# iosefa/obia

Measured on AMD Instinct MI355X. Metric: Mpixel/s (SLIC+zonal feats) on 16384²×8-band; achieved HBM GB/s fraction, higher is better.
Workload: dtype f32

## Files before the change

obia_amd/csrc/slic.hip:

```cpp
#include "slic.hpp"
#include "slic_features.hpp"

#include <cmath>
#include <cstdlib>

namespace obia {

void regular_grid_hw(long long H, long long W, long long n, long long out[4]) {
    long long dims[3] = {1, H, W};
    int order[3] = {0, 1, 2};
    for (int i = 0; i < 3; ++i)
        for (int j = i + 1; j < 3; ++j)
            if (dims[order[j]] < dims[order[i]]) std::swap(order[i], order[j]);
    double sd[3];
    for (int i = 0; i < 3; ++i) sd[i] = (double)dims[order[i]];
    double space = sd[0] * sd[1] * sd[2];
    if (space <= (double)n) { out[0] = out[1] = out[2] = out[3] = 0; return; }
    double st[3];
    for (int i = 0; i < 3; ++i) st[i] = std::pow(space / (double)n, 1.0 / 3.0);
    auto all_ge = [&]() { return sd[0] >= st[0] && sd[1] >= st[1] && sd[2] >= st[2]; };
    if (!all_ge()) {
        for (int d = 0; d < 3; ++d) {
            st[d] = sd[d];
            double sp = 1.0;
// ... 688 lines not shown
    __syncthreads();
    if (threadIdx.x == 0) {
        const int tot = s_c[0] + s_c[1] + s_c[2] + s_c[3];
        if (tot) atomicAdd(&out[p], tot);
    }
}

int slic_plan_layout(obia_ctx *ctx, SlicBatch &b) {
    if (b.d_tile_prob) return OBIA_OK;
    const int np = b.nprob;
    long long tiles_all = 0;
    int tile_max = 0;
    for (int p = 0; p < np; ++p) {
        SlicProblem &P = b.probs[p];
        P.tiles_x = cdiv(P.W, SWEEP_TW);
        P.tiles_y = cdiv(P.H, SWEEP_TH);
        const int nt = P.tiles_x * P.tiles_y;
        if (tiles_all + nt > 0x7fff0000LL) { set_error("too many sweep tiles in one batch"); return OBIA_E_INVALID; }
        P.tile_off = (int)tiles_all;
        tiles_all += nt;
        if (nt > tile_max) tile_max = nt;
    }
    b.total_tiles_all = tiles_all > 0 ? tiles_all : 1;
    b.total_tiles = tile_max;
    std::vector<int> tp((size_t)b.total_tiles_all, 0);
    for (int p = 0; p < np; ++p)
        for (int t = 0; t < b.probs[p].tiles_x * b.probs[p].tiles_y; ++t) tp[(size_t)b.probs[p].tile_off + t] = p;
    b.d_probs = ctx->plan.add(ctx, b.probs.data(), (size_t)np);
    b.d_tile_prob = ctx->plan.add(ctx, tp.data(), tp.size());
    if (!b.d_probs || !b.d_tile_prob) return OBIA_E_NOMEM;
    return OBIA_OK;
}

int slic_count_valid(obia_ctx *ctx, SlicBatch &b, std::vector<int> &nvalid, int *d_cnt_cleared) {
    const int np = b.nprob;
    Arena &A = ctx->arena;
    nvalid.assign(np, 0);
    OBIA_TRY(slic_plan_layout(ctx, b));
    if (b.masked) {
        OBIA_TRY(ctx->plan.flush(ctx));
        int *d_cnt = d_cnt_cleared;
        if (!d_cnt) {
            d_cnt = A.get<int>(np);
            if (!d_cnt) return OBIA_E_NOMEM;
            OBIA_TRY(fill_async(ctx, d_cnt, 0, sizeof(int) * np));
        }
        int blocks = cdiv(b.maxpix, 256 * 16 * 32);
        if (blocks < 1) blocks = 1;
        hipLaunchKernelGGL(count_valid_kernel, dim3(blocks, np), dim3(256), 0, ctx->stream, b.d_probs, b.d_mask, d_cnt);
        OBIA_TRY(read_back(ctx, nvalid.data(), d_cnt, sizeof(int) * np));
    } else {
        for (int p = 0; p < np; ++p) nvalid[p] = b.probs[p].H * b.probs[p].W;
    }
    return OBIA_OK;
}

int slic_plan_and_seed(obia_ctx *ctx, SlicBatch &b, const std::vector<int> &n_segments, const std::vector<int> *nvalid_in,
                       const ExternalSeeds *ext) {
    const int np = b.nprob;
    if (ext)
        for (int p = 0; p < np; ++p)
            if (ext[p].n < 0 || (ext[p].n > 0 && !ext[p].yx && !ext[p].d_yx)) { set_error("external seeds of problem %d: bad set", p); return OBIA_E_INVALID; }
    Arena &A = ctx->arena;
    OBIA_TRY(slic_plan_layout(ctx, b));
    std::vector<int> nvalid;
    if (nvalid_in) nvalid = *nvalid_in;
    else OBIA_TRY(slic_count_valid(ctx, b, nvalid));
    if (ext && np == 1 && ext->n > 0 && nvalid[0] <= 0) { set_error("the mask has no valid pixel"); return OBIA_E_EMPTY; }
    std::vector<SeedGrid> grids(np);
    std::vector<double> stepmax(np);
    b.step.assign(np, 1.0f);
    b.grid_n.assign(np, 0);
    int cent_off = 0;
    for (int p = 0; p < np; ++p) {
// ... 149 lines not shown
```

obia_amd/csrc/slic.hpp:

```cpp
#pragma once
#include "common.hpp"

namespace obia {

struct SlicProblem {
    int H, W;
    int K;
    int sy, sx;
    int ncy, ncx;
    float spatial_w;
    int cent_off;
    int cell_off;
    int tile_off;
    int tiles_x, tiles_y;
    long long pix_off;
    long long feat_off;
    int XB;
    int n_valid;
    long long fb_off;
    float sp_y, sp_x;
    int direct;
    int m4_off;
};

// ... 101 lines not shown
    }
    return members;
}

struct SmoothSpec {
    double sigma[3] = {0.0, 0.0, 0.0};
    float *tmp_a = nullptr, *tmp_b = nullptr;
    double *d_w[3] = {nullptr, nullptr, nullptr};
    int radius[3] = {0, 0, 0};
    unsigned *d_scratch = nullptr;
    bool on() const { return sigma[0] > 1e-15 || sigma[1] > 1e-15 || sigma[2] > 1e-15; }
};
int smooth_prepare(obia_ctx *ctx, SmoothSpec &sm, long long total_pix, int CP, int np);
int gaussian_weights_host(double sigma, bool sigma_is_f32, std::vector<double> &w);
int slic_features_launch(hipStream_t stream, const SlicBatch &b, const float *src, int Ws, unsigned *d_keys, const SmoothSpec *smooth = nullptr,
                         bool minmax_only = false);
bool slic_fuse_features(const SlicBatch &b, const float *src, int Ws);
double slic_fscale(float maxabs);
int slic_features_finish(SlicBatch &b, const unsigned *keys, const unsigned *nonfinite, const unsigned *maxabs_bits, std::vector<int> *skip);
int slic_prepare_features(obia_ctx *ctx, SlicBatch &b, const float *src, int Ws, std::vector<int> *skip = nullptr);
float slic_prescale(float ratio, int normalize, int to_lab, bool slic_zero);
bool slic_use_colour_bound(float ratio, bool to_lab = false);
void slic_batch_settings(SlicBatch &b, const obia_slic_params &p, int C, int normalize_bands, bool masked);
int slic_batch_layout(SlicBatch &b);
inline std::pair<int, int> slic_cc_sizes(double min_size_factor, double max_size_factor, int n_valid, int K) {
    const double segment_size = K > 0 ? (double)n_valid / (double)K : 1.0;
    const double mxd = max_size_factor * segment_size;
    return {(int)(min_size_factor * segment_size), mxd >= 2147483647.0 ? 2147483647 : (mxd >= 1.0 ? (int)mxd : 1)};
}

struct ExternalSeeds { const double *yx; int n; double step; const float *d_yx = nullptr; };
int slic_plan_and_seed(obia_ctx *ctx, SlicBatch &b, const std::vector<int> &n_segments,
                       const std::vector<int> *nvalid = nullptr, const ExternalSeeds *ext = nullptr);
int slic_count_valid(obia_ctx *ctx, SlicBatch &b, std::vector<int> &nvalid, int *d_cnt_cleared = nullptr);
int slic_plan_layout(obia_ctx *ctx, SlicBatch &b);

int slic_run_sweeps(obia_ctx *ctx, SlicBatch &b);
int slic_sweeps_settle(obia_ctx *ctx, bool *repeat);
int slic_rerun_storing(obia_ctx *ctx, SlicBatch &b);

int slic_stage_outputs(obia_ctx *ctx, const SlicBatch &b, float *features, float *seeds_yx, float *centroids);

int mask_centroids_dev(obia_ctx *ctx, const uint8_t *mask, int H, int W, const int64_t *picks, int K, const int64_t *dense, long long n_dense,
                       int iters, double *centroids_yx_out, double *steps_zyx_out);
int mask_centroids_queue(obia_ctx *ctx, const uint8_t *mask, int h, int w, long long n_valid, const int64_t *picks, int K, const int64_t *dense,
                         long long n_dense, int iters, float *seeds_out_dev, double *steps_out_dev);

struct CcProblem { int H, W; long long pix_off; int min_size; int max_size; };
struct CcResolve { const int *parent; const int *newlab; const int *small_final; int start_label; int mask_label; };
#if defined(__HIPCC__)
__device__ __forceinline__ int cc_resolve_label(const CcResolve &R, long long i) {
    const int p = R.parent[i];
    if (p < 0) return R.mask_label;
    const int r = R.parent[p];
    int nl = R.newlab[r];
    if (nl < 0) nl = R.small_final[-nl - 2];
    return (nl >= 0) ? nl + R.start_label : 0;
}
#endif
int enforce_connectivity_batch(obia_ctx *ctx, const std::vector<CcProblem> &probs, const int32_t *labels_in,
                               long long total_pix, int start_label, int32_t *labels_out, int *h_n_labels_out,
                               CcResolve *deferred = nullptr, const CcProblem *d_probs = nullptr);

int enforce_connectivity_dev(obia_ctx *ctx, const int32_t *labels_in, int H, int W, int min_size,
                             int max_size, int start_label, int32_t *labels_out, int *d_n_labels_out);

int zonal_stats_dev(obia_ctx *ctx, const float *raw, const int32_t *labels, int H, int W, int C,
                    const int32_t *bands_host, int n_bands, int n_labels, int start_label,
                    int64_t *count, double *mean, double *var, float *mn, float *mx);
int zonal_moments_dev(obia_ctx *ctx, const float *raw, const int32_t *labels, int H, int W, int C,
                      const int32_t *bands_host, int n_bands, int n_labels, int start_label, const double *mean,
                      double *skew, double *kurt, double *var );

}
```

obia_amd/csrc/tiling.hip:

```cpp
#include "slic.hpp"
#include "../../include/obia_testing.h"

#include <cmath>
#include <cstdlib>

namespace obia {

struct TileWin { int y0, x0, h, w; long long pix_off; int cly, clx; int cly_in, clx_in, cly_any, clx_any; int m4_off; };

__device__ __forceinline__ void wave_hist_add(unsigned *hist, int key, bool active) {
    bool todo = active;
    while (true) {
        const unsigned long long act = __ballot(todo);
        if (!act) break;
        const int leader = __ffsll((long long)act) - 1;
        const int kk = __shfl(key, leader);
        const unsigned long long same = __ballot(todo && key == kk);
        if ((int)(threadIdx.x & 63) == leader) atomicAdd(&hist[kk], (unsigned)__popcll(same));
        if (key == kk) todo = false;
    }
}

__device__ __forceinline__ bool in_corner(const TileWin &t, int y, int x) {
    return (y >= t.h - t.cly) && (x < t.clx || x >= t.w - t.clx);
}
__device__ __forceinline__ bool wholly_in_corner(const TileWin &t, int y, int x) {
    return (y >= t.h - t.cly_in) && (x < t.clx_in || x >= t.w - t.clx_in);
}
__device__ __forceinline__ bool meets_corner(const TileWin &t, int y, int x) {
    return (y >= t.h - t.cly_any) && (x < t.clx_any || x >= t.w - t.clx_any);
}

__global__ __launch_bounds__(256) void tile_count_inside_kernel(const TileWin *__restrict__ wins, const int32_t *__restrict__ G,
                                                                int Wr, unsigned *__restrict__ inside, int *__restrict__ tile_any) {
    const TileWin t = wins[blockIdx.y];
    bool seen = false;
    const int wround = ((t.w + 255) / 256) * 256;
    for (int y = blockIdx.x; y < t.h; y += gridDim.x) {
        const bool low = y >= t.h - t.cly_any;
        for (int x0 = 0; x0 < wround; x0 += 4 * 256) {
            int g[4];
#pragma unroll
            for (int u = 0; u < 4; ++u) {
                const int x = x0 + 256 * u + threadIdx.x;
                g[u] = 0;
                if (x < t.w && !(low && wholly_in_corner(t, y, x))) {
                    g[u] = G[(long long)(t.y0 + y) * Wr + t.x0 + x];
                    seen |= g[u] > 0;
                    if (low && meets_corner(t, y, x)) g[u] = 0;
                }
            }
#pragma unroll
            for (int u = 0; u < 4; ++u)
                if (x0 + 256 * u < wround) wave_hist_add(inside, g[u], g[u] > 0);
        }
    }
    if (__ballot(seen) && (threadIdx.x & 63) == 0) tile_any[blockIdx.y] = 1;
}

template <bool VEC4>
__global__ __launch_bounds__(256) void tile_mask_kernel(const TileWin *__restrict__ wins, const uint8_t *__restrict__ inmask,
                                                        int32_t *__restrict__ G, int Wr, int white,
                                                        const unsigned *__restrict__ inside, const unsigned *__restrict__ seg_size,
                                                        uint8_t *__restrict__ alive, uint8_t *__restrict__ dmask,
                                                        const int *__restrict__ tile_any, unsigned *__restrict__ dmask4) {
    const TileWin t = wins[blockIdx.y];
    if (white && tile_any[blockIdx.y] == 0) white = 0;
    auto decide = [&](int y, int x, long long gp, uint8_t m, int g) -> uint8_t {
        if (!white) return m;
        if (in_corner(t, y, x)) return 0;
        if (g > 0) {
            if (inside[g] == seg_size[g]) { G[gp] = 0; alive[g] = 0; }
            else m = 0;
        }
        return m;
    };
    if (VEC4) {
        const int w4 = t.w >> 2, nq = (t.h + 3) >> 2;
        for (int q = blockIdx.x; q < nq; q += gridDim.x)
            for (int x4 = threadIdx.x; x4 < w4; x4 += 256) {
                const int x = 4 * x4;
                unsigned mw[4];
                int4 g[4];
#pragma unroll
                for (int j = 0; j < 4; ++j) {
                    const int y = 4 * q + j;
                    const long long gp = (long long)(t.y0 + (y < t.h ? y : t.h - 1)) * Wr + t.x0 + x;
                    mw[j] = inmask ? *reinterpret_cast<const unsigned *>(inmask + gp) : 0x01010101u;
                    g[j] = make_int4(0, 0, 0, 0);
                    if (white) g[j] = *reinterpret_cast<const int4 *>(G + gp);
                }
                unsigned out[4] = {0u, 0u, 0u, 0u};
#pragma unroll
                for (int j = 0; j < 4; ++j) {
                    const int y = 4 * q + j;
                    if (y >= t.h) continue;
                    const long long gp = (long long)(t.y0 + y) * Wr + t.x0 + x;
                    const int gv[4] = {g[j].x, g[j].y, g[j].z, g[j].w};
#pragma unroll
                    for (int u = 0; u < 4; ++u) {
                        const uint8_t m = ((mw[j] >> (8 * u)) & 0xffu) != 0;
                        out[j] |= (unsigned)decide(y, x + u, gp + u, m, gv[u]) << (8 * u);
                    }
                    *reinterpret_cast<unsigned *>(dmask + t.pix_off + (long long)y * t.w + x) = out[j];
                }
                uint4 o;
                unsigned *ov = &o.x;
#pragma unroll
                for (int c = 0; c < 4; ++c)
                    ov[c] = ((out[0] >> (8 * c)) & 0xffu) | (((out[1] >> (8 * c)) & 0xffu) << 8) | (((out[2] >> (8 * c)) & 0xffu) << 16) |
                            (((out[3] >> (8 * c)) & 0xffu) << 24);
                *reinterpret_cast<uint4 *>(dmask4 + (long long)t.m4_off + (long long)q * t.w + x) = o;
            }
        return;
    }
    for (int y = blockIdx.x; y < t.h; y += gridDim.x)
    for (int x0 = threadIdx.x; x0 < t.w; x0 += 4 * 256) {
        uint8_t mv[4];
        int gv[4];
#pragma unroll
        for (int u = 0; u < 4; ++u) {
            const int x = x0 + 256 * u;
            mv[u] = 0; gv[u] = 0;
            if (x < t.w) {
                const long long gp = (long long)(t.y0 + y) * Wr + t.x0 + x;
                mv[u] = inmask ? (inmask[gp] != 0) : 1;
                if (white && !in_corner(t, y, x)) gv[u] = G[gp];
            }
        }
#pragma unroll
        for (int u = 0; u < 4; ++u) {
            const int x = x0 + 256 * u;
            if (x >= t.w) continue;
            const long long gp = (long long)(t.y0 + y) * Wr + t.x0 + x;
            dmask[t.pix_off + (long long)y * t.w + x] = decide(y, x, gp, mv[u], gv[u]);
        }
    }
}

constexpr int TS_SLOTS = 128;
__global__ __launch_bounds__(64) void tile_scatter_kernel(const TileWin *__restrict__ wins, const CcResolve R,
                                                          int32_t *__restrict__ G, int Wr, int id_base,
                                                          unsigned *__restrict__ seg_size) {
    __shared__ int s_key[TS_SLOTS];
    __shared__ unsigned s_cnt[TS_SLOTS];
    const TileWin t = wins[blockIdx.y];
    const int bw = (t.w + 63) / 64;
    const int by = blockIdx.x / bw, bx = blockIdx.x % bw;
    if (by * 64 >= t.h) return;
    const int lane = threadIdx.x;
    for (int i = lane; i < TS_SLOTS; i += 64) { s_key[i] = 0; s_cnt[i] = 0; }
    __syncthreads();
    const int x = bx * 64 + lane;
    const bool col_ok = x < t.w;
    const int y_lo = by * 64, y_hi = min(y_lo + 64, t.h);
    int rid = 0;
    unsigned rn = 0;
    auto close_run = [&]() {
        if (rid <= 0) return;
        const unsigned h = ((unsigned)rid * 2654435761u) >> 25;
        int slot = -1;
#pragma unroll 1
        for (int probe = 0; probe < TS_SLOTS; ++probe) {
            const int sidx = (h + probe) & (TS_SLOTS - 1);
            const int old = atomicCAS(&s_key[sidx], 0, rid);
            if (old == 0 || old == rid) { slot = sidx; break; }
        }
        if (slot >= 0) atomicAdd(&s_cnt[slot], rn);
        else atomicAdd(&seg_size[rid], rn);
    };
#pragma unroll 1
    for (int y0 = y_lo; y0 < y_hi; y0 += 8) {
        int l[8];
#pragma unroll
        for (int j = 0; j < 8; ++j) {
            const int y = y0 + j;
            l[j] = (col_ok && y < y_hi) ? cc_resolve_label(R, t.pix_off + (long long)y * t.w + x) : 0;
        }
#pragma unroll
        for (int j = 0; j < 8; ++j) {
            const int y = y0 + j;
            const int id = l[j] > 0 ? id_base + l[j] : 0;
            if (id > 0) G[(long long)(t.y0 + y) * Wr + t.x0 + x] = id;
            if (id != rid) { close_run(); rid = id; rn = 0; }
            rn += 1;
        }
    }
    close_run();
    __syncthreads();
    for (int i = lane; i < TS_SLOTS; i += 64)
        if (s_key[i] > 0 && s_cnt[i]) atomicAdd(&seg_size[s_key[i]], s_cnt[i]);
}

constexpr int IDS_CHUNK = 1024 * 16;

__global__ __launch_bounds__(1024) void ids_count_kernel(const uint8_t *__restrict__ alive, int n_ids, int *__restrict__ partial) {
    __shared__ int s_wave[16];
    const int tid = threadIdx.x, lane = tid & 63, wv = tid >> 6;
    const int i0 = blockIdx.x * IDS_CHUNK + tid * 16;
    int c = 0;
#pragma unroll
    for (int q = 0; q < 16; ++q) c += (i0 + q < n_ids) ? (alive[i0 + q] != 0) : 0;
#pragma unroll
    for (int off = 32; off > 0; off >>= 1) c += __shfl_xor(c, off);
    if (lane == 0) s_wave[wv] = c;
    __syncthreads();
    if (tid == 0) {
        int t = 0;
        for (int w2 = 0; w2 < 16; ++w2) t += s_wave[w2];
        partial[blockIdx.x] = t;
    }
}

__global__ __launch_bounds__(1024) void ids_scan_kernel(const uint8_t *__restrict__ alive, int n_ids, const int *__restrict__ partial,
                                                        int *__restrict__ newid, long long *__restrict__ total) {
    __shared__ int s_wave[16];
    __shared__ int s_base[16];
    const int tid = threadIdx.x, lane = tid & 63, wv = tid >> 6;
    int pre = 0;
    for (int j = tid; j < (int)blockIdx.x; j += 1024) pre += partial[j];
#pragma unroll
// ... 16 lines not shown
    __syncthreads();
    int before = 0;
    for (int w2 = 0; w2 < 16; ++w2) { before += s_base[w2]; if (w2 < wv) before += s_wave[w2]; }
    int run = before + inc - c;
#pragma unroll
    for (int q = 0; q < 16; ++q)
        if (i0 + q < n_ids) { if (f[q]) { run += 1; newid[i0 + q] = run; } else newid[i0 + q] = 0; }
    if (blockIdx.x == gridDim.x - 1 && tid == 1023) *total = before + inc;
}

__global__ __launch_bounds__(256) void ids_apply_kernel(int32_t *__restrict__ G, long long n, const int *__restrict__ newid) {
    const long long n4 = ((reinterpret_cast<uintptr_t>(G) & 15) == 0) ? n / 4 : 0;
    int4 *G4 = reinterpret_cast<int4 *>(G);
    for (long long i = (long long)blockIdx.x * blockDim.x + threadIdx.x; i < n4; i += (long long)gridDim.x * blockDim.x) {
        int4 g = G4[i];
        g.x = g.x > 0 ? newid[g.x] : 0;
        g.y = g.y > 0 ? newid[g.y] : 0;
        g.z = g.z > 0 ? newid[g.z] : 0;
        g.w = g.w > 0 ? newid[g.w] : 0;
        G4[i] = g;
    }
    for (long long i = n4 * 4 + (long long)blockIdx.x * blockDim.x + threadIdx.x; i < n; i += (long long)gridDim.x * blockDim.x) {
        const int g = G[i];
        G[i] = g > 0 ? newid[g] : 0;
    }
}

struct TileState {
    int H, W, C;
    int Hg, row0;
    const float *img;
    const uint8_t *inmask;
    int32_t *G;
    unsigned *seg_size, *inside;
    uint8_t *alive;
    int *newid;
    long long *d_total;
    int id_cap, next_id;
    int clx, cly, clx_in, cly_in, clx_any, cly_any;
    obia_tiling_params tp;
    obia_slic_params sp;
    SlicBatch settings;
    int seeding = OBIA_SEEDING_GRID;
    obia_pick_fn pick_fn = nullptr;
    void *pick_user = nullptr;
    struct PreFeat {
        bool ready = false;
        bool planned = false;
        bool fused = false;
        SlicBatch b;
        std::vector<unsigned> host;
        unsigned *d_keys = nullptr;
        bool launched = false;
        bool on_side = false;
        size_t cursor = 0;
    } pf;
};


static int grid_rows(const std::vector<TileWin> &wins) {
    int g = 1;
    for (auto &t : wins) if (t.h > g) g = t.h;
    return (int)grids::tiler_rows(g, 1).x.n;
}

#ifndef OBIA_PREFETCH_BESIDE
// ... 70 lines not shown
    b.d_mask = A.get<uint8_t>((size_t)b.total_pix);
    unsigned *d_mask4 = A.get<unsigned>((size_t)b.total_m4);
    if (!d_mask4) return OBIA_E_NOMEM;
    const bool pre = white && S.pf.ready;
    if (pre) {
        const SlicBatch &pb = S.pf.b;
        if (S.pf.cursor + np > pb.windows.size()) { set_error("white batch beyond the prefetched windows"); return OBIA_E_INVALID; }
        const SrcWindow *a = &pb.windows[S.pf.cursor];
        for (int p = 0; p < np; ++p)
            if (a[p].y0 != wins[p].y0 || a[p].x0 != wins[p].x0 || a[p].h != wins[p].h || a[p].w != wins[p].w) { set_error("white batch does not match the prefetched windows"); return OBIA_E_INVALID; }
        if (S.pf.fused) {
            b.d_feat = A.get<float>(4 * (size_t)b.total_feat_f4);
            b.fuse_features = true;
            b.raw_src = S.img; b.raw_ws = S.W;
            b.d_keys = S.pf.d_keys + S.pf.cursor * (size_t)S.C * 2;
        } else {
            b.d_feat = pb.d_feat + 4 * (size_t)a[0].feat_off;
            if (b.col_lb) b.d_fbox = pb.d_fbox + (size_t)a[0].fb_off * 2 * b.CP;
        }
    } else {
        b.d_feat = A.get<float>(4 * (size_t)b.total_feat_f4);
        if (b.col_lb) {
            b.d_fbox = A.get<float>((size_t)b.total_boxes * 2 * b.CP);
            if (!b.d_fbox) return OBIA_E_NOMEM;
        }
    }
    b.d_labels = A.get<int32_t>((size_t)b.total_pix);
    if (!b.d_mask || !b.d_feat || !b.d_labels) return OBIA_E_NOMEM;
    TileWin *d_wins = ctx->plan.add(ctx, wins.data(), (size_t)np);
    b.d_windows = ctx->plan.add(ctx, b.windows.data(), (size_t)np);
    if (!d_wins || !b.d_windows) return OBIA_E_NOMEM;
    OBIA_TRY(slic_plan_layout(ctx, b));
    OBIA_TRY(ctx->plan.flush(ctx));
    int *d_tile_any = A.get<int>(np), *d_cnt = A.get<int>(np);
    if (!d_tile_any || !d_cnt) return OBIA_E_NOMEM;
    {
        ClearSet clr(ctx);
        if (white) {
            OBIA_TRY(clr.add(S.inside, 0, sizeof(unsigned) * (size_t)S.next_id));
            OBIA_TRY(clr.add(d_tile_any, 0, sizeof(int) * (size_t)np));
        }
        OBIA_TRY(clr.add(d_cnt, 0, sizeof(int) * (size_t)np));
        OBIA_TRY(clr.flush());
    }
    if (white) {
        hipLaunchKernelGGL(tile_count_inside_kernel, dim3(grid_rows(wins), np), dim3(256), 0, ctx->stream, d_wins, S.G, S.W, S.inside, d_tile_any);
    }
    {
        bool vec4 = (S.W % 4 == 0) && (reinterpret_cast<uintptr_t>(S.inmask) % 4 == 0) && (reinterpret_cast<uintptr_t>(S.G) % 16 == 0) &&
                    (reinterpret_cast<uintptr_t>(b.d_mask) % 4 == 0) && (reinterpret_cast<uintptr_t>(d_mask4) % 16 == 0);
        for (auto &t : wins) vec4 = vec4 && (t.x0 % 4 == 0) && (t.w % 4 == 0) && (t.pix_off % 4 == 0);
        if (vec4) {
            hipLaunchKernelGGL(HIP_KERNEL_NAME(tile_mask_kernel<true>), dim3((grid_rows(wins) + 3) / 4, np), dim3(256), 0, ctx->stream, d_wins, S.inmask,
                               S.G, S.W, white ? 1 : 0, S.inside, S.seg_size, S.alive, b.d_mask, d_tile_any, d_mask4);
            b.d_mask4 = d_mask4;
        } else {
            hipLaunchKernelGGL(HIP_KERNEL_NAME(tile_mask_kernel<false>), dim3(grid_rows(wins), np), dim3(256), 0, ctx->stream, d_wins, S.inmask,
                               S.G, S.W, white ? 1 : 0, S.inside, S.seg_size, S.alive, b.d_mask, d_tile_any, d_mask4);
        }
    }
    std::vector<int> skip;
    if (pre) {
        const size_t NP = S.pf.b.windows.size(), nkeys = NP * (size_t)S.C * 2;
        const unsigned *h = S.pf.host.data();
        OBIA_TRY(slic_features_finish(b, h + S.pf.cursor * (size_t)S.C * 2, h + nkeys + S.pf.cursor, h + nkeys + NP + S.pf.cursor, &skip));
        S.pf.cursor += np;
    } else {
        OBIA_TRY(slic_prepare_features(ctx, b, S.img, S.W, &skip));
    }
    std::vector<int> nvalid;
    debug_sync(ctx, "tiler: mask + features");
    OBIA_TRY(slic_count_valid(ctx, b, nvalid, d_cnt));
    debug_sync(ctx, "tiler: count_valid");
    std::vector<int> nseg(np);
    const double pixel_area = S.tp.pixel_width * S.tp.pixel_height;
    const double crown_area = M_PI * S.tp.crown_radius * S.tp.crown_radius;
    for (int p = 0; p < np; ++p) {
        double n;
        if (S.sp.n_segments > 0)
            n = std::nearbyint((double)S.sp.n_segments * (double)nvalid[p] / ((double)S.tp.tile_size * S.tp.tile_size));
        else
            n = std::nearbyint((double)nvalid[p] * pixel_area / crown_area);
        nseg[p] = (skip[p] || n < 1.0) ? 0 : (n > 2.0e9 ? 2000000000 : (int)n);
    }
    std::vector<ExternalSeeds> ext;
    if (S.seeding == OBIA_SEEDING_SKIMAGE) OBIA_TRY(seed_tiles_skimage(ctx, S, b, nvalid, nseg, ext));
    OBIA_TRY(slic_plan_and_seed(ctx, b, nseg, &nvalid, ext.empty() ? nullptr : ext.data()));
    debug_sync(ctx, "tiler: plan_and_seed");
    std::vector<CcProblem> cps(np);
    for (int p = 0; p < np; ++p) {
        const SlicProblem &P = b.probs[p];
        const auto [min_size, max_size] = slic_cc_sizes(S.sp.min_size_factor, S.sp.max_size_factor, P.n_valid, P.K);
        cps[p] = CcProblem{P.H, P.W, P.pix_off, min_size, max_size};
    }
    const CcProblem *d_cps = S.sp.enforce_connectivity ? ctx->plan.add(ctx, cps.data(), (size_t)np) : nullptr;
    if (S.sp.enforce_connectivity && !d_cps) return OBIA_E_NOMEM;
    if (!white && S.pf.planned && !S.pf.launched)
        OBIA_TRY(prefetch_white_launch(ctx, S, OBIA_PREFETCH_BESIDE != 0 || b.exit_on_fixed_point || b.slic_zero));
    const Arena::Mark sweeps_mk = A.mark();
    unsigned *const mask4 = b.d_mask4;
    OBIA_TRY(slic_run_sweeps(ctx, b));
    debug_sync(ctx, "tiler: sweeps");
    int n_new = 0;
    CcResolve resolve{};
    if (S.sp.enforce_connectivity) {
        OBIA_TRY(enforce_connectivity_batch(ctx, cps, b.d_labels, b.total_pix, 1, nullptr, &n_new, &resolve, d_cps));
        bool repeat = false;
        OBIA_TRY(slic_sweeps_settle(ctx, &repeat));
        if (repeat) {
            A.rewind(sweeps_mk);
            b.d_mask4 = mask4;
            OBIA_TRY(slic_rerun_storing(ctx, b));
            OBIA_TRY(enforce_connectivity_batch(ctx, cps, b.d_labels, b.total_pix, 1, nullptr, &n_new, &resolve, d_cps));
            OBIA_TRY(slic_sweeps_settle(ctx, nullptr));
        }
        debug_sync(ctx, "tiler: connectivity");
    } else {
        set_error("the tiled driver needs enforce_connectivity=True (segments must be connected pixel sets)");
        return OBIA_E_UNSUPPORTED;
    }
    if (S.next_id + n_new > S.id_cap) { set_error("segment id capacity exceeded (%d + %d > %d)", S.next_id, n_new, S.id_cap); return OBIA_E_NOMEM; }
    if (n_new > 0) {
        int sblocks = 1;
        for (auto &t : wins) sblocks = std::max(sblocks, cdiv(t.w, 64) * cdiv(t.h, 64));
        hipLaunchKernelGGL(tile_scatter_kernel, dim3(sblocks, np), dim3(64), 0, ctx->stream, d_wins, resolve, S.G, S.W,
                           S.next_id - 1, S.seg_size);
        OBIA_TRY(fill_async(ctx, S.alive + S.next_id, 1, (size_t)n_new));
        S.next_id += n_new;
    }
    OBIA_HIP_TRY(hipGetLastError());
    OBIA_TRY(ctx->plan.flush(ctx));
    A.rewind(mk);
    return OBIA_OK;
}

__global__ __launch_bounds__(256) void seam_mark_kernel(const int32_t *__restrict__ codes, int n, int me, int owner, int32_t *__restrict__ fmap,
                                                        int cap, int *__restrict__ new_list, int *__restrict__ ctr, int32_t *__restrict__ ids) {
    int tmax = 0;
    for (int i = blockIdx.x * blockDim.x + threadIdx.x; i < n; i += gridDim.x * blockDim.x) {
        const int c = codes[i];
        int id = 0;
        if (c > 0) {
            const int o = (c >> 24) - 1, t = c & 0xffffff;
            if (o == me) id = t;
            else if (o == owner) {
                tmax = max(tmax, t);
                if (t > 0 && t < cap) {
                    const int f = fmap[t];
                    if (f > 0) id = f;
                    else if (f == 0 && atomicCAS(&fmap[t], 0, -1) == 0) new_list[atomicAdd(&ctr[0], 1)] = t;
                }
            }
        }
        ids[i] = id;
    }
    for (int off = 32; off > 0; off >>= 1) tmax = max(tmax, __shfl_xor(tmax, off));
    if ((threadIdx.x & 63) == 0 && tmax > 0) atomicMax(&ctr[1], tmax);
}
constexpr int SEAM_SORT = 16384;
// ... 40 lines not shown
        const int t = c & 0xffffff;
        if (t > 0 && t < cap) ids[i] = fmap[t];
    }
}
__global__ __launch_bounds__(256) void seam_unclaim_kernel(const int *__restrict__ new_list, int m, int32_t *__restrict__ fmap) {
    for (int i = blockIdx.x * blockDim.x + threadIdx.x; i < m; i += gridDim.x * blockDim.x) fmap[new_list[i]] = 0;
}
__global__ void seam_register_kernel(unsigned *__restrict__ seg_size, uint8_t *__restrict__ alive, int first, int count) {
    const int i = blockIdx.x * blockDim.x + threadIdx.x;
    if (i < count) { seg_size[first + i] = 0xffffffffu; alive[first + i] = 1; }
}

static int tiler_check(const float *img, int H, int W, int C, int Hg, int row0, const obia_tiling_params *tp,
                       const obia_slic_params *sp, const int32_t *labels) {
    if (!img || !tp || !sp || !labels) { set_error("null argument"); return OBIA_E_INVALID; }
    if (H <= 0 || W <= 0 || C <= 0 || C > 16) { set_error("bad raster shape (%d,%d,%d)", H, W, C); return OBIA_E_INVALID; }
    if (row0 < 0 || row0 + H > Hg) { set_error("local rows [%d,%d) outside the global raster of %d rows", row0, row0 + H, Hg); return OBIA_E_INVALID; }
    if ((long long)H * W > 0x7fffffffLL) { set_error("raster above 2^31 pixels: shard it across GPUs"); return OBIA_E_INVALID; }
    if (tp->tile_size <= 0 || tp->buffer < 0) { set_error("tile_size must be positive and buffer non-negative"); return OBIA_E_INVALID; }
    if (!(sp->compactness > 0.0) || sp->max_num_iter < 0) { set_error("bad SLIC parameters"); return OBIA_E_INVALID; }
    for (int i = 0; i < 3; ++i) {
        if (!(sp->sigma_zyx[i] >= 0.0)) { set_error("sigma must be >= 0"); return OBIA_E_INVALID; }
        if (!(sp->spacing_zyx[i] > 0.0) || !(sp->spacing_zyx[i] < 1.0e30)) { set_error("spacing must be positive and finite"); return OBIA_E_INVALID; }
    }
    if (!sp->enforce_connectivity) { set_error("the tiled driver needs enforce_connectivity=True (segments must be connected pixel sets)"); return OBIA_E_UNSUPPORTED; }
    if (sp->n_segments <= 0 && !(tp->crown_radius > 0.0 && tp->pixel_width > 0.0 && tp->pixel_height > 0.0)) {
        set_error("crown_radius and pixel size must be positive when n_segments is not given");
        return OBIA_E_INVALID;
    }
    return OBIA_OK;
}

static int tiler_init(obia_ctx *ctx, TileState &S, const float *img, const uint8_t *mask, int H, int W, int C, int Hg,
                      int row0, const obia_tiling_params *tp, const obia_slic_params *sp, int32_t *labels, int extra_ids) {
    OBIA_TRY(tiler_check(img, H, W, C, Hg, row0, tp, sp, labels));
    const int T = tp->tile_size, B = tp->buffer;
    Arena &A = ctx->arena;
    const int ntx = cdiv(W, T), nty = cdiv(H, T) + 2;
    const double pixel_area = tp->pixel_width * tp->pixel_height;
    const double crown_area = M_PI * tp->crown_radius * tp->crown_radius;
    const long long wh = (long long)(T + 2 * B) * (T + 2 * B);
    double n = sp->n_segments > 0 ? (double)sp->n_segments * (double)wh / ((double)T * T) : (double)wh * pixel_area / crown_area;
    if (n < 1) n = 1;
    long long cap = (long long)(n * 1.5 + 64.0) * (long long)ntx * nty + 16 + extra_ids;
    if (cap > 0x7ffffff0LL) { set_error("too many segments for int32 ids"); return OBIA_E_INVALID; }
    S.H = H; S.W = W; S.C = C; S.Hg = Hg; S.row0 = row0; S.img = img; S.inmask = mask; S.G = labels; S.tp = *tp; S.sp = *sp;
    S.id_cap = (int)cap; S.next_id = 1;
    slic_batch_settings(S.settings, *sp, C, 1, true);
    S.settings.start_label = 1;
    S.seg_size = A.get<unsigned>((size_t)cap);
    S.inside = A.get<unsigned>((size_t)cap);
    S.alive = A.get<uint8_t>((size_t)cap);
    S.newid = A.get<int>((size_t)cap);
    S.d_total = A.get<long long>(1);
    if (!S.seg_size || !S.inside || !S.alive || !S.newid || !S.d_total) return OBIA_E_NOMEM;
    OBIA_TRY(fill_async(ctx, S.seg_size, 0, sizeof(unsigned) * (size_t)cap));
    OBIA_TRY(fill_async(ctx, S.alive, 0, (size_t)cap));
    S.clx = S.cly = S.clx_in = S.cly_in = S.clx_any = S.cly_any = 0;
    if (B > 0) {
        const double cl = (double)B / 2.0;
        auto count = [](double px, double cl, int kind) {
            if (!(px > 0.0)) px = 1.0;
            long long k = (long long)std::floor(cl / px) + 2;
            if (k < 0) k = 0;
            auto holds = [&](long long i) { return kind == 0 ? (i + 0.5) * px < cl : (kind == 1 ? (i + 1.0) * px <= cl : i * px < cl); };
            while (k > 0 && !holds(k - 1)) --k;
            return (int)std::min<long long>(k, 0x3fffffff);
        };
        S.clx = count(tp->pixel_width, cl, 0);  S.cly = count(tp->pixel_height, cl, 0);
        S.clx_in = count(tp->pixel_width, cl, 1);  S.cly_in = count(tp->pixel_height, cl, 1);
        S.clx_any = count(tp->pixel_width, cl, 2);  S.cly_any = count(tp->pixel_height, cl, 2);
    }
    return OBIA_OK;
}

static TileWin white_window(const TileState &S, int tj, int ti) {
    const int T = S.tp.tile_size, B = S.tp.buffer;
    const int y0 = std::max(0, tj * T - B), y1 = std::min(S.Hg, tj * T + T + B);
    const int x0 = std::max(0, ti * T - B), x1 = std::min(S.W, ti * T + T + B);
    const int h = y1 - y0, w = x1 - x0;
    return TileWin{y0 - S.row0, x0, h, w, 0, std::min(S.cly, h), std::min(S.clx, w), std::min(S.cly_in, h), std::min(S.clx_in, w),
                   std::min(S.cly_any, h), std::min(S.clx_any, w), 0};
}

static int prefetch_white_plan(obia_ctx *ctx, TileState &S, int white_order) {
    const int T = S.tp.tile_size;
    const int ntx = cdiv(S.W, T), nty = cdiv(S.Hg, T);
    TileState::PreFeat &pf = S.pf;
    pf = TileState::PreFeat();
    if (S.sp.sigma_zyx[0] > 0.0 || S.sp.sigma_zyx[1] > 0.0 || S.sp.sigma_zyx[2] > 0.0) return OBIA_OK;
// ... 92 lines not shown
        }
        if (white && per_row) OBIA_TRY(flush());
    }
    if (!wins.empty()) OBIA_TRY(flush());
    return OBIA_OK;
}

static int tiler_finalize(obia_ctx *ctx, TileState &S, int64_t *n_segments_out) {
    const int nchunks = cdiv(S.next_id, IDS_CHUNK);
    int *d_partial = ctx->arena.get<int>((size_t)nchunks);
    if (!d_partial) return OBIA_E_NOMEM;
    hipLaunchKernelGGL(ids_count_kernel, dim3(nchunks), dim3(1024), 0, ctx->stream, S.alive, S.next_id, d_partial);
    hipLaunchKernelGGL(ids_scan_kernel, dim3(nchunks), dim3(1024), 0, ctx->stream, S.alive, S.next_id, d_partial, S.newid, S.d_total);
    const int g = (int)grids::tiler_ids_apply((long long)S.H * S.W).x.n;
    hipLaunchKernelGGL(ids_apply_kernel, dim3(g), dim3(256), 0, ctx->stream, S.G, (long long)S.H * S.W, S.newid);
    OBIA_HIP_TRY(hipGetLastError());
    long long total = 0;
    OBIA_TRY(read_back(ctx, &total, S.d_total, sizeof(long long)));
    if (n_segments_out) *n_segments_out = total;
    return OBIA_OK;
}

static int check_seeding(int seeding, obia_pick_fn picks) {
    if (seeding != OBIA_SEEDING_GRID && seeding != OBIA_SEEDING_SKIMAGE) { set_error("seeding must be OBIA_SEEDING_GRID or OBIA_SEEDING_SKIMAGE (got %d)", seeding); return OBIA_E_INVALID; }
    if (seeding == OBIA_SEEDING_SKIMAGE && !picks) { set_error("seeding = skimage needs a pick function"); return OBIA_E_INVALID; }
    return OBIA_OK;
}

static int tiled_slic_dev(obia_ctx *ctx, const float *img, const uint8_t *mask, int H, int W, int C,
                          const obia_tiling_params *tp, const obia_slic_params *sp, int seeding, obia_pick_fn picks, void *picks_user,
                          int32_t *labels_out, int64_t *n_segments_out) {
    TileState S;
    OBIA_TRY(check_seeding(seeding, picks));
    OBIA_TRY(tiler_init(ctx, S, img, mask, H, W, C, H, 0, tp, sp, labels_out, 0));
    S.seeding = seeding; S.pick_fn = picks; S.pick_user = picks_user;
    OBIA_TRY(fill_async(ctx, labels_out, 0, sizeof(int32_t) * (size_t)H * W));
    const int nty = cdiv(H, tp->tile_size);
    OBIA_TRY(prefetch_white_plan(ctx, S, tp->white_order));
    OBIA_TRY(tiler_run(ctx, S, false, 0, nty, -1));
    if (std::getenv("OBIA_DEBUG_FAIL_AFTER_BLACK")) {
        set_error("debug: forced failure after the black pass");
        return OBIA_E_INVALID;
    }
    OBIA_TRY(prefetch_white_fetch(ctx, S));
    if (tp->white_order == 1) {
        OBIA_TRY(tiler_run(ctx, S, true, 0, nty, 0));
        OBIA_TRY(tiler_run(ctx, S, true, 0, nty, 1));
    } else {
        OBIA_TRY(tiler_run(ctx, S, true, 0, nty, -1));
    }
    return tiler_finalize(ctx, S, n_segments_out);
}

}

struct obia_tiler {
    obia_ctx *ctx;
    obia::TileState S;
    int *seam_buf = nullptr;
    size_t seam_cap = 0;
};

using namespace obia;

static int enter(obia_tiler *t) {
    if (!t) { set_error("null tiler"); return OBIA_E_INVALID; }
    return enter(t->ctx, t);
// ... 166 lines not shown
```

Baseline: 7672.

## Track written label blocks in an occupancy bitmap to skip empty reads in tiler

Adds a per-64x64-block occupancy bitmap over the global label image, set by the scatter kernel when it writes labels. The count-inside and mask kernels consult it to skip loading G from blocks never written, and the count-inside kernel is restructured to iterate per occupancy block. The mask kernel now also produces per-block nonzero counts, which removes the separate count_valid kernel launch. The scatter kernel skips repeated label resolution when the parent matches the previous row. The costs are extra atomics, more per-pixel bitmap tests, and a larger readback of partial counts.

```diff
diff --git a/obia_amd/csrc/slic.hip b/obia_amd/csrc/slic.hip
--- a/obia_amd/csrc/slic.hip
+++ b/obia_amd/csrc/slic.hip
@@ -744,7 +744,7 @@
     return OBIA_OK;
 }
 
-int slic_count_valid(obia_ctx *ctx, SlicBatch &b, std::vector<int> &nvalid, int *d_cnt_cleared) {
+int slic_count_valid(obia_ctx *ctx, SlicBatch &b, std::vector<int> &nvalid, int *d_cnt_cleared, int counted_parts) {
     const int np = b.nprob;
     Arena &A = ctx->arena;
     nvalid.assign(np, 0);
@@ -752,6 +752,14 @@
     if (b.masked) {
         OBIA_TRY(ctx->plan.flush(ctx));
         int *d_cnt = d_cnt_cleared;
+        if (counted_parts > 0) {
+            if (!d_cnt) { set_error("slic_count_valid: counts announced without their buffer"); return OBIA_E_INVALID; }
+            std::vector<int> parts((size_t)np * counted_parts);
+            OBIA_TRY(read_back(ctx, parts.data(), d_cnt, sizeof(int) * parts.size()));
+            for (int p = 0; p < np; ++p)
+                for (int q = 0; q < counted_parts; ++q) nvalid[p] += parts[(size_t)p * counted_parts + q];
+            return OBIA_OK;
+        }
         if (!d_cnt) {
             d_cnt = A.get<int>(np);
             if (!d_cnt) return OBIA_E_NOMEM;
diff --git a/obia_amd/csrc/slic.hpp b/obia_amd/csrc/slic.hpp
--- a/obia_amd/csrc/slic.hpp
+++ b/obia_amd/csrc/slic.hpp
@@ -157,7 +157,7 @@
 struct ExternalSeeds { const double *yx; int n; double step; const float *d_yx = nullptr; };
 int slic_plan_and_seed(obia_ctx *ctx, SlicBatch &b, const std::vector<int> &n_segments,
                        const std::vector<int> *nvalid = nullptr, const ExternalSeeds *ext = nullptr);
-int slic_count_valid(obia_ctx *ctx, SlicBatch &b, std::vector<int> &nvalid, int *d_cnt_cleared = nullptr);
+int slic_count_valid(obia_ctx *ctx, SlicBatch &b, std::vector<int> &nvalid, int *d_cnt_cleared = nullptr, int counted_parts = 0);
 int slic_plan_layout(obia_ctx *ctx, SlicBatch &b);
 
 int slic_run_sweeps(obia_ctx *ctx, SlicBatch &b);
@@ -174,14 +174,14 @@
 struct CcProblem { int H, W; long long pix_off; int min_size; int max_size; };
 struct CcResolve { const int *parent; const int *newlab; const int *small_final; int start_label; int mask_label; };
 #if defined(__HIPCC__)
-__device__ __forceinline__ int cc_resolve_label(const CcResolve &R, long long i) {
-    const int p = R.parent[i];
+__device__ __forceinline__ int cc_resolve_parent(const CcResolve &R, int p) {
     if (p < 0) return R.mask_label;
     const int r = R.parent[p];
     int nl = R.newlab[r];
     if (nl < 0) nl = R.small_final[-nl - 2];
     return (nl >= 0) ? nl + R.start_label : 0;
 }
+__device__ __forceinline__ int cc_resolve_label(const CcResolve &R, long long i) { return cc_resolve_parent(R, R.parent[i]); }
 #endif
 int enforce_connectivity_batch(obia_ctx *ctx, const std::vector<CcProblem> &probs, const int32_t *labels_in,
                                long long total_pix, int start_label, int32_t *labels_out, int *h_n_labels_out,
diff --git a/obia_amd/csrc/tiling.hip b/obia_amd/csrc/tiling.hip
--- a/obia_amd/csrc/tiling.hip
+++ b/obia_amd/csrc/tiling.hip
@@ -31,29 +31,46 @@
     return (y >= t.h - t.cly_any) && (x < t.clx_any || x >= t.w - t.clx_any);
 }
 
+constexpr int OCC_SHIFT = 6;
+__device__ __forceinline__ bool occ_test(const unsigned *__restrict__ occ, int occ_bw, int gy, int gx) {
+    if (!occ) return true;
+    const int b = (gy >> OCC_SHIFT) * occ_bw + (gx >> OCC_SHIFT);
+    return (occ[b >> 5] >> (b & 31)) & 1u;
+}
+
+constexpr int COUNT_ROWS_PER_WAVE = (1 << OCC_SHIFT) / 4;
 __global__ __launch_bounds__(256) void tile_count_inside_kernel(const TileWin *__restrict__ wins, const int32_t *__restrict__ G,
-                                                                int Wr, unsigned *__restrict__ inside, int *__restrict__ tile_any) {
+                                                                int Wr, unsigned *__restrict__ inside, int *__restrict__ tile_any,
+                                                                const unsigned *__restrict__ occ, int occ_bw) {
     const TileWin t = wins[blockIdx.y];
+    const int cb0 = t.x0 >> OCC_SHIFT, rb0 = t.y0 >> OCC_SHIFT;
+    const int nbx = ((t.x0 + t.w - 1) >> OCC_SHIFT) - cb0 + 1, nby = ((t.y0 + t.h - 1) >> OCC_SHIFT) - rb0 + 1;
+    if ((int)blockIdx.x >= nbx * nby) return;
+    const int rb = rb0 + (int)blockIdx.x / nbx, cb = cb0 + (int)blockIdx.x % nbx;
+    if (!occ_test(occ, occ_bw, rb << OCC_SHIFT, cb << OCC_SHIFT)) return;
+    const int wv = __builtin_amdgcn_readfirstlane((int)(threadIdx.x >> 6));
+    const int x = (cb << OCC_SHIFT) + (int)(threadIdx.x & 63) - t.x0;
+    const bool col_ok = x >= 0 && x < t.w;
+    const int y_first = (rb << OCC_SHIFT) + wv * COUNT_ROWS_PER_WAVE - t.y0;
     bool seen = false;
-    const int wround = ((t.w + 255) / 256) * 256;
-    for (int y = blockIdx.x; y < t.h; y += gridDim.x) {
-        const bool low = y >= t.h - t.cly_any;
-        for (int x0 = 0; x0 < wround; x0 += 4 * 256) {
-            int g[4];
-#pragma unroll
-            for (int u = 0; u < 4; ++u) {
-                const int x = x0 + 256 * u + threadIdx.x;
-                g[u] = 0;
-                if (x < t.w && !(low && wholly_in_corner(t, y, x))) {
-                    g[u] = G[(long long)(t.y0 + y) * Wr + t.x0 + x];
-                    seen |= g[u] > 0;
-                    if (low && meets_corner(t, y, x)) g[u] = 0;
-                }
+#pragma unroll 1
+    for (int yb = y_first; yb < y_first + COUNT_ROWS_PER_WAVE; yb += 8) {
+        int g[8];
+#pragma unroll
+        for (int j = 0; j < 8; ++j) {
+            const int y = yb + j;
+            g[j] = 0;
+            if (y < 0 || y >= t.h) continue;
+            const bool low = y >= t.h - t.cly_any;
+            if (col_ok && !(low && wholly_in_corner(t, y, x))) {
+                g[j] = G[(long long)(t.y0 + y) * Wr + t.x0 + x];
+                seen |= g[j] > 0;
+                if (low && meets_corner(t, y, x)) g[j] = 0;
             }
-#pragma unroll
-            for (int u = 0; u < 4; ++u)
-                if (x0 + 256 * u < wround) wave_hist_add(inside, g[u], g[u] > 0);
-        }
+        }
+#pragma unroll
+        for (int j = 0; j < 8; ++j)
+            if (yb + j >= 0 && yb + j < t.h) wave_hist_add(inside, g[j], g[j] > 0);
     }
     if (__ballot(seen) && (threadIdx.x & 63) == 0) tile_any[blockIdx.y] = 1;
 }
@@ -63,8 +80,18 @@
                                                         int32_t *__restrict__ G, int Wr, int white,
                                                         const unsigned *__restrict__ inside, const unsigned *__restrict__ seg_size,
                                                         uint8_t *__restrict__ alive, uint8_t *__restrict__ dmask,
-                                                        const int *__restrict__ tile_any, unsigned *__restrict__ dmask4) {
+                                                        const int *__restrict__ tile_any, unsigned *__restrict__ dmask4,
+                                                        const unsigned *__restrict__ occ, int occ_bw, int *__restrict__ parts) {
     const TileWin t = wins[blockIdx.y];
+    __shared__ int s_nz[4];
+    int nz = 0;
+    auto store_count = [&]() {
+#pragma unroll
+        for (int off = 32; off > 0; off >>= 1) nz += __shfl_xor(nz, off);
+        if ((threadIdx.x & 63) == 0) s_nz[threadIdx.x >> 6] = nz;
+        __syncthreads();
+        if (threadIdx.x == 0) parts[(size_t)blockIdx.y * gridDim.x + blockIdx.x] = s_nz[0] + s_nz[1] + s_nz[2] + s_nz[3];
+    };
     if (white && tile_any[blockIdx.y] == 0) white = 0;
     auto decide = [&](int y, int x, long long gp, uint8_t m, int g) -> uint8_t {
         if (!white) return m;
@@ -82,13 +109,15 @@
                 const int x = 4 * x4;
                 unsigned mw[4];
                 int4 g[4];
+                const bool load_g = white && (occ_test(occ, occ_bw, t.y0 + 4 * q, t.x0 + x) || occ_test(occ, occ_bw, t.y0 + min(4 * q + 3, t.h - 1), t.x0 + x));
 #pragma unroll
                 for (int j = 0; j < 4; ++j) {
                     const int y = 4 * q + j;
-                    const long long gp = (long long)(t.y0 + (y < t.h ? y : t.h - 1)) * Wr + t.x0 + x;
+                    const int gy = t.y0 + (y < t.h ? y : t.h - 1);
+                    const long long gp = (long long)gy * Wr + t.x0 + x;
                     mw[j] = inmask ? *reinterpret_cast<const unsigned *>(inmask + gp) : 0x01010101u;
                     g[j] = make_int4(0, 0, 0, 0);
-                    if (white) g[j] = *reinterpret_cast<const int4 *>(G + gp);
+                    if (load_g) g[j] = *reinterpret_cast<const int4 *>(G + gp);
                 }
                 unsigned out[4] = {0u, 0u, 0u, 0u};
 #pragma unroll
@@ -103,6 +132,7 @@
                         out[j] |= (unsigned)decide(y, x + u, gp + u, m, gv[u]) << (8 * u);
                     }
                     *reinterpret_cast<unsigned *>(dmask + t.pix_off + (long long)y * t.w + x) = out[j];
+                    nz += __popc(out[j]);
                 }
                 uint4 o;
                 unsigned *ov = &o.x;
@@ -112,6 +142,7 @@
                             (((out[3] >> (8 * c)) & 0xffu) << 24);
                 *reinterpret_cast<uint4 *>(dmask4 + (long long)t.m4_off + (long long)q * t.w + x) = o;
             }
+        store_count();
         return;
     }
     for (int y = blockIdx.x; y < t.h; y += gridDim.x)
@@ -125,7 +156,7 @@
             if (x < t.w) {
                 const long long gp = (long long)(t.y0 + y) * Wr + t.x0 + x;
                 mv[u] = inmask ? (inmask[gp] != 0) : 1;
-                if (white && !in_corner(t, y, x)) gv[u] = G[gp];
+                if (white && !in_corner(t, y, x) && occ_test(occ, occ_bw, t.y0 + y, t.x0 + x)) gv[u] = G[gp];
             }
         }
 #pragma unroll
@@ -133,15 +164,18 @@
             const int x = x0 + 256 * u;
             if (x >= t.w) continue;
             const long long gp = (long long)(t.y0 + y) * Wr + t.x0 + x;
-            dmask[t.pix_off + (long long)y * t.w + x] = decide(y, x, gp, mv[u], gv[u]);
-        }
-    }
+            const uint8_t m = decide(y, x, gp, mv[u], gv[u]);
+            dmask[t.pix_off + (long long)y * t.w + x] = m;
+            nz += m;
+        }
+    }
+    store_count();
 }
 
 constexpr int TS_SLOTS = 128;
 __global__ __launch_bounds__(64) void tile_scatter_kernel(const TileWin *__restrict__ wins, const CcResolve R,
                                                           int32_t *__restrict__ G, int Wr, int id_base,
-                                                          unsigned *__restrict__ seg_size) {
+                                                          unsigned *__restrict__ seg_size, unsigned *__restrict__ occ, int occ_bw) {
     __shared__ int s_key[TS_SLOTS];
     __shared__ unsigned s_cnt[TS_SLOTS];
     const TileWin t = wins[blockIdx.y];
@@ -169,24 +203,54 @@
         if (slot >= 0) atomicAdd(&s_cnt[slot], rn);
         else atomicAdd(&seg_size[rid], rn);
     };
+    const int rb0 = (t.y0 + y_lo) >> OCC_SHIFT;
+    const int y_split = ((rb0 + 1) << OCC_SHIFT) - t.y0;
+    bool wrote0 = false, wrote1 = false;
+    int p_above = -1, l_above = R.mask_label;
 #pragma unroll 1
     for (int y0 = y_lo; y0 < y_hi; y0 += 8) {
-        int l[8];
+        int par[8], l[8];
 #pragma unroll
         for (int j = 0; j < 8; ++j) {
             const int y = y0 + j;
-            l[j] = (col_ok && y < y_hi) ? cc_resolve_label(R, t.pix_off + (long long)y * t.w + x) : 0;
-        }
+            par[j] = (col_ok && y < y_hi) ? R.parent[t.pix_off + (long long)y * t.w + x] : -1;
+        }
+        unsigned fresh = 0;
+#pragma unroll
+        for (int j = 0; j < 8; ++j) {
+            l[j] = R.mask_label;
+            if (par[j] >= 0 && par[j] != (j ? par[j - 1] : p_above)) { l[j] = cc_resolve_parent(R, par[j]); fresh |= 1u << j; }
+        }
+#pragma unroll
+        for (int j = 0; j < 8; ++j)
+            if (par[j] >= 0 && !((fresh >> j) & 1u)) l[j] = j ? l[j - 1] : l_above;
+        p_above = par[7]; l_above = l[7];
 #pragma unroll
         for (int j = 0; j < 8; ++j) {
             const int y = y0 + j;
-            const int id = l[j] > 0 ? id_base + l[j] : 0;
-            if (id > 0) G[(long long)(t.y0 + y) * Wr + t.x0 + x] = id;
+            const int id = (col_ok && y < y_hi && l[j] > 0) ? id_base + l[j] : 0;
+            if (id > 0) {
+                G[(long long)(t.y0 + y) * Wr + t.x0 + x] = id;
+                if (y >= y_split) wrote1 = true; else wrote0 = true;
+            }
             if (id != rid) { close_run(); rid = id; rn = 0; }
             rn += 1;
         }
     }
     close_run();
+    if (occ) {
+        const int cb0 = (t.x0 + bx * 64) >> OCC_SHIFT;
+#pragma unroll
+        for (int r = 0; r < 2; ++r)
+#pragma unroll
+            for (int c = 0; c < 2; ++c) {
+                const bool mine = (r ? wrote1 : wrote0) && ((t.x0 + x) >> OCC_SHIFT) == cb0 + c;
+                if (__ballot(mine) && lane == 0) {
+                    const int b = (rb0 + r) * occ_bw + cb0 + c;
+                    if (!((occ[b >> 5] >> (b & 31)) & 1u)) atomicOr(&occ[b >> 5], 1u << (b & 31));
+                }
+            }
+    }
     __syncthreads();
     for (int i = lane; i < TS_SLOTS; i += 64)
         if (s_key[i] > 0 && s_cnt[i]) atomicAdd(&seg_size[s_key[i]], s_cnt[i]);
@@ -269,6 +333,8 @@
     const float *img;
     const uint8_t *inmask;
     int32_t *G;
+    unsigned *occ = nullptr;
+    int occ_bw = 0;
     unsigned *seg_size, *inside;
     uint8_t *alive;
     int *newid;
@@ -405,32 +471,29 @@
     if (!d_wins || !b.d_windows) return OBIA_E_NOMEM;
     OBIA_TRY(slic_plan_layout(ctx, b));
     OBIA_TRY(ctx->plan.flush(ctx));
-    int *d_tile_any = A.get<int>(np), *d_cnt = A.get<int>(np);
+    bool vec4 = (S.W % 4 == 0) && (reinterpret_cast<uintptr_t>(S.inmask) % 4 == 0) && (reinterpret_cast<uintptr_t>(S.G) % 16 == 0) &&
+                (reinterpret_cast<uintptr_t>(b.d_mask) % 4 == 0) && (reinterpret_cast<uintptr_t>(d_mask4) % 16 == 0);
+    for (auto &t : wins) vec4 = vec4 && (t.x0 % 4 == 0) && (t.w % 4 == 0) && (t.pix_off % 4 == 0);
+    const int mask_grid = vec4 ? (grid_rows(wins) + 3) / 4 : grid_rows(wins);
+    int *d_tile_any = A.get<int>(np), *d_cnt = A.get<int>((size_t)np * mask_grid);
     if (!d_tile_any || !d_cnt) return OBIA_E_NOMEM;
-    {
+    if (white) {
         ClearSet clr(ctx);
-        if (white) {
-            OBIA_TRY(clr.add(S.inside, 0, sizeof(unsigned) * (size_t)S.next_id));
-            OBIA_TRY(clr.add(d_tile_any, 0, sizeof(int) * (size_t)np));
-        }
-        OBIA_TRY(clr.add(d_cnt, 0, sizeof(int) * (size_t)np));
+        OBIA_TRY(clr.add(S.inside, 0, sizeof(unsigned) * (size_t)S.next_id));
+        OBIA_TRY(clr.add(d_tile_any, 0, sizeof(int) * (size_t)np));
         OBIA_TRY(clr.flush());
-    }
-    if (white) {
-        hipLaunchKernelGGL(tile_count_inside_kernel, dim3(grid_rows(wins), np), dim3(256), 0, ctx->stream, d_wins, S.G, S.W, S.inside, d_tile_any);
-    }
-    {
-        bool vec4 = (S.W % 4 == 0) && (reinterpret_cast<uintptr_t>(S.inmask) % 4 == 0) && (reinterpret_cast<uintptr_t>(S.G) % 16 == 0) &&
-                    (reinterpret_cast<uintptr_t>(b.d_mask) % 4 == 0) && (reinterpret_cast<uintptr_t>(d_mask4) % 16 == 0);
-        for (auto &t : wins) vec4 = vec4 && (t.x0 % 4 == 0) && (t.w % 4 == 0) && (t.pix_off % 4 == 0);
-        if (vec4) {
-            hipLaunchKernelGGL(HIP_KERNEL_NAME(tile_mask_kernel<true>), dim3((grid_rows(wins) + 3) / 4, np), dim3(256), 0, ctx->stream, d_wins, S.inmask,
-                               S.G, S.W, white ? 1 : 0, S.inside, S.seg_size, S.alive, b.d_mask, d_tile_any, d_mask4);
-            b.d_mask4 = d_mask4;
-        } else {
-            hipLaunchKernelGGL(HIP_KERNEL_NAME(tile_mask_kernel<false>), dim3(grid_rows(wins), np), dim3(256), 0, ctx->stream, d_wins, S.inmask,
-                               S.G, S.W, white ? 1 : 0, S.inside, S.seg_size, S.alive, b.d_mask, d_tile_any, d_mask4);
-        }
+        int cblocks = 1;
+        for (auto &t : wins) cblocks = std::max(cblocks, (cdiv(t.w, 1 << OCC_SHIFT) + 1) * (cdiv(t.h, 1 << OCC_SHIFT) + 1));
+        hipLaunchKernelGGL(tile_count_inside_kernel, dim3(cblocks, np), dim3(256), 0, ctx->stream, d_wins, S.G, S.W, S.inside, d_tile_any, S.occ,
+                           S.occ_bw);
+    }
+    if (vec4) {
+        hipLaunchKernelGGL(HIP_KERNEL_NAME(tile_mask_kernel<true>), dim3(mask_grid, np), dim3(256), 0, ctx->stream, d_wins, S.inmask,
+                           S.G, S.W, white ? 1 : 0, S.inside, S.seg_size, S.alive, b.d_mask, d_tile_any, d_mask4, S.occ, S.occ_bw, d_cnt);
+        b.d_mask4 = d_mask4;
+    } else {
+        hipLaunchKernelGGL(HIP_KERNEL_NAME(tile_mask_kernel<false>), dim3(mask_grid, np), dim3(256), 0, ctx->stream, d_wins, S.inmask,
+                           S.G, S.W, white ? 1 : 0, S.inside, S.seg_size, S.alive, b.d_mask, d_tile_any, d_mask4, S.occ, S.occ_bw, d_cnt);
     }
     std::vector<int> skip;
     if (pre) {
@@ -443,7 +506,7 @@
     }
     std::vector<int> nvalid;
     debug_sync(ctx, "tiler: mask + features");
-    OBIA_TRY(slic_count_valid(ctx, b, nvalid, d_cnt));
+    OBIA_TRY(slic_count_valid(ctx, b, nvalid, d_cnt, mask_grid));
     debug_sync(ctx, "tiler: count_valid");
     std::vector<int> nseg(np);
     const double pixel_area = S.tp.pixel_width * S.tp.pixel_height;
@@ -497,7 +560,7 @@
         int sblocks = 1;
         for (auto &t : wins) sblocks = std::max(sblocks, cdiv(t.w, 64) * cdiv(t.h, 64));
         hipLaunchKernelGGL(tile_scatter_kernel, dim3(sblocks, np), dim3(64), 0, ctx->stream, d_wins, resolve, S.G, S.W,
-                           S.next_id - 1, S.seg_size);
+                           S.next_id - 1, S.seg_size, S.occ, S.occ_bw);
         OBIA_TRY(fill_async(ctx, S.alive + S.next_id, 1, (size_t)n_new));
         S.next_id += n_new;
     }
@@ -604,7 +667,8 @@
 }
 
 static int tiler_init(obia_ctx *ctx, TileState &S, const float *img, const uint8_t *mask, int H, int W, int C, int Hg,
-                      int row0, const obia_tiling_params *tp, const obia_slic_params *sp, int32_t *labels, int extra_ids) {
+                      int row0, const obia_tiling_params *tp, const obia_slic_params *sp, int32_t *labels, int extra_ids,
+                      bool occupancy = false) {
     OBIA_TRY(tiler_check(img, H, W, C, Hg, row0, tp, sp, labels));
     const int T = tp->tile_size, B = tp->buffer;
     Arena &A = ctx->arena;
@@ -628,6 +692,14 @@
     if (!S.seg_size || !S.inside || !S.alive || !S.newid || !S.d_total) return OBIA_E_NOMEM;
     OBIA_TRY(fill_async(ctx, S.seg_size, 0, sizeof(unsigned) * (size_t)cap));
     OBIA_TRY(fill_async(ctx, S.alive, 0, (size_t)cap));
+    S.occ = nullptr;
+    S.occ_bw = cdiv(W, 1 << OCC_SHIFT);
+    if (occupancy) {
+        const size_t words = ((size_t)S.occ_bw * (size_t)cdiv(H, 1 << OCC_SHIFT) + 31) / 32;
+        S.occ = A.get<unsigned>(words);
+        if (!S.occ) return OBIA_E_NOMEM;
+        OBIA_TRY(fill_async(ctx, S.occ, 0, sizeof(unsigned) * words));
+    }
     S.clx = S.cly = S.clx_in = S.cly_in = S.clx_any = S.cly_any = 0;
     if (B > 0) {
         const double cl = (double)B / 2.0;
@@ -786,7 +858,8 @@
                           int32_t *labels_out, int64_t *n_segments_out) {
     TileState S;
     OBIA_TRY(check_seeding(seeding, picks));
-    OBIA_TRY(tiler_init(ctx, S, img, mask, H, W, C, H, 0, tp, sp, labels_out, 0));
+    const char *occ_env = std::getenv("OBIA_G_OCCUPANCY");
+    OBIA_TRY(tiler_init(ctx, S, img, mask, H, W, C, H, 0, tp, sp, labels_out, 0, !(occ_env && occ_env[0] == '0')));
     S.seeding = seeding; S.pick_fn = picks; S.pick_user = picks_user;
     OBIA_TRY(fill_async(ctx, labels_out, 0, sizeof(int32_t) * (size_t)H * W));
     const int nty = cdiv(H, tp->tile_size);
```

New measurement: 7806, median of 6. 1.7% higher.
